# ashishkumar822/Jetson-SLAM

Hardware: AMD Instinct MI355X
Metric: stereo pairs/s (FAST+ORB extract L+R + stereo match) (higher is better)
Workload: dtype u8/int32 (+f32 orientation/blur)

## Files before the change

jetson_slam_amd/csrc/k_stereo.hip:

```cpp
#include <algorithm>
#include <cstdlib>

#include "jsorb_launch.h"

namespace jsorb {

__device__ __forceinline__ int hamming256(const uint4 a0, const uint4 a1, const uint4 b0, const uint4 b1)
{
    return __popc(a0.x ^ b0.x) + __popc(a0.y ^ b0.y) + __popc(a0.z ^ b0.z) + __popc(a0.w ^ b0.w) +
           __popc(a1.x ^ b1.x) + __popc(a1.y ^ b1.y) + __popc(a1.z ^ b1.z) + __popc(a1.w ^ b1.w);
}

#define SKPW 4
#define SGL (64 / SKPW)

__device__ __forceinline__ void wave_lds_sync_st()
{
    __builtin_amdgcn_fence(__ATOMIC_RELEASE, "wavefront");
    __builtin_amdgcn_wave_barrier();
    __builtin_amdgcn_fence(__ATOMIC_ACQUIRE, "wavefront");
}

#define ST_MAX_PASS 8
#define ST_MAX_KP (SKPW * ST_MAX_PASS)
#ifndef ST_MIN_WAVES
#define ST_MIN_WAVES 5
#endif
__global__ __launch_bounds__(64, ST_MIN_WAVES) void k_stereo(Geometry g, ImageSrc srcL, const uint8_t *slabL, ImageSrc srcR, const uint8_t *slabR,
                                               const int32_t *__restrict__ outL, const int *__restrict__ countsL, const uint8_t *__restrict__ descL,
                                               const int32_t *__restrict__ outR, const int *__restrict__ countsR, const uint8_t *__restrict__ descR,
                                               const int *__restrict__ row_tabR,
                                               float *__restrict__ u_right, float *__restrict__ depth, int *__restrict__ best_l1,
                                               unsigned *__restrict__ aux, StereoArgs sa, int n_pairs, int *__restrict__ diag, int npass)
{
    __shared__ int s_lvi[JSORB_MAX_LEVELS][12];
    __shared__ float s_lvf[JSORB_MAX_LEVELS][2];
    __shared__ unsigned s_best[ST_MAX_KP];
    __shared__ int s_ncand[ST_MAX_KP];
    __shared__ __align__(16) unsigned s_par[ST_MAX_KP][8];
    __shared__ __align__(16) unsigned s_ctr[ST_MAX_KP][4];
    __shared__ __align__(16) unsigned s_acc[ST_MAX_KP][8];
    const int lane = threadIdx.x;
    const int grp = lane / SGL, sl = lane % SGL;
    const int kpw = SKPW * npass;
    int b, blk;
    if (!xcd_map((g.T + kpw - 1) / kpw, n_pairs, b, blk)) return;
    const int Nl = uniform_i32(countsL[b * (JSORB_MAX_LEVELS + 1) + JSORB_MAX_LEVELS]);
    const int Nr = uniform_i32(countsR[b * (JSORB_MAX_LEVELS + 1) + JSORB_MAX_LEVELS]);
    if (blk * kpw >= Nl) return;
    if (lane < g.L) {
        const LevelDesc &lv = g.lv[lane];
        s_lvi[lane][3] = lv.W; s_lvi[lane][4] = lv.pitch; s_lvi[lane][5] = (int)lv.img_off;
        if (!g.epi_rows) {
            s_lvi[lane][0] = lv.th; s_lvi[lane][1] = lv.nth; s_lvi[lane][2] = lv.row_tab_off;
            s_lvi[lane][6] = (int)(0xFFFFFFFFu / (unsigned)lv.th + 1u);
            s_lvi[lane][7] = lv.tw; s_lvi[lane][8] = lv.ntw; s_lvi[lane][9] = lv.tile_off;
            s_lvi[lane][10] = (int)(0xFFFFFFFFu / (unsigned)lv.tw + 1u);
        }
        s_lvf[lane][0] = lv.scale; s_lvf[lane][1] = lv.inv_scale;
    }
    if (lane < ST_MAX_KP) { s_best[lane] = 0xFFFFFFFFu; s_ncand[lane] = 0; }
    reinterpret_cast<uint4 *>(s_acc)[lane] = make_uint4(0, 0, 0, 0);
    static_assert(ST_MAX_KP * 8 * 4 == 64 * 16, "one 16-byte store per lane clears the L1 counters");
    wave_lds_sync_st();
    const int32_t *oL = outL + (size_t)b * 6 * g.T;
    const int32_t *oR = outR + (size_t)b * 6 * g.T;
    const size_t tb = (size_t)b * g.T;

    struct LeftKp { int x, y, level; uint4 a0, a1; };
    auto load_left = [&](int pass) {
        const int i = min(blk * kpw + pass * SKPW + grp, Nl - 1);
        const uint4 *dl = reinterpret_cast<const uint4 *>(descL + (tb + i) * 32);
        return LeftKp{oL[i], oL[Nl + i], oL[4 * (size_t)Nl + i], dl[0], dl[1]};
    };
#ifndef ST_PREFETCH
#define ST_PREFETCH 1
#endif
#if ST_PREFETCH
    LeftKp nxt = load_left(0);
#endif
    for (int pass = 0; pass < npass; pass++) {
        if (blk * kpw + pass * SKPW >= Nl) break;
        const int i_raw = blk * kpw + pass * SKPW + grp;
        const bool live = i_raw < Nl;
#if ST_PREFETCH
        const LeftKp cur = nxt;
        nxt = load_left(pass + 1);
#else
        const LeftKp cur = load_left(pass);
#endif
        const int levelL = cur.level;
        const float uL = (float)cur.x, vL = (float)cur.y;
        const float minU = uL - sa.maxD, maxU = uL - 0.0f;
        unsigned best_key = 0xFFFFFFFFu;
        int n_cand = 0;
        {
            const uint4 a0 = cur.a0, a1 = cur.a1;
            const int vLi = (int)vL;
            const int *rt = row_tabR + (size_t)b * g.row_tab_stride;
            if (g.epi_rows) {
                const int EH = g.epi_rows, EN = g.L * EH;
                const int *et = rt + g.epi_off;
                const int2 *ee = reinterpret_cast<const int2 *>(et + ((EN + 2) & ~1));
                int seg_start = 0, seg_len = 0;
                {
                    const int lr = levelL - 1 + sl;
                    if (sl < 3 && lr >= 0 && lr < g.L && !(maxU < 0)) {
                        const float r = 2.0f * s_lvf[lr][0], vLf = (float)vLi;
                        const float lo_f = __builtin_floorf(vLf - 2.0f - r), hi_f = __builtin_ceilf(vLf + 2.0f + r);
                        int below = 0, above = 0;
#pragma unroll
                        for (int k = 0; k < 5; k++) {
                            below += __builtin_ceilf((lo_f + (float)k) + r) < vLf ? 1 : 0;
                            above += __builtin_floorf((hi_f - (float)k) - r) > vLf ? 1 : 0;
                        }
                        const int ylo = max((int)lo_f + below, 0), yhi = min((int)hi_f - above, EH - 1);
                        if (ylo <= yhi) {
                            seg_start = et[lr * EH + ylo];
                            seg_len = et[lr * EH + yhi + 1] - seg_start;
                        }
                    }
                }
                const int gl0 = lane & ~(SGL - 1);
                const int st0 = __shfl(seg_start, gl0, 64), st1 = __shfl(seg_start, gl0 + 1, 64), st2 = __shfl(seg_start, gl0 + 2, 64);
                const int c1 = __shfl(seg_len, gl0, 64), c2 = c1 + __shfl(seg_len, gl0 + 1, 64), total = c2 + __shfl(seg_len, gl0 + 2, 64);
#ifndef ST_CAND_UNROLL
#define ST_CAND_UNROLL 3
#endif
                constexpr int CU = ST_CAND_UNROLL;
                for (int k = sl; k < total; k += CU * SGL) {
                    int2 e[CU];
                    bool ok[CU];
#pragma unroll
                    for (int u = 0; u < CU; u++) {
                        const int kk = k + u * SGL;
                        const int kc = kk < total ? kk : k;
                        e[u] = ee[(kc >= c2 ? st2 - c2 : (kc >= c1 ? st1 - c1 : st0)) + kc];
                    }
                    uint4 b0[CU], b1[CU];
#pragma unroll
                    for (int u = 0; u < CU; u++) {
                        const float uR = (float)(e[u].y & 0xFFFF);
                        ok[u] = k + u * SGL < total && uR >= minU && uR <= maxU;
                        const uint4 *dr = reinterpret_cast<const uint4 *>(descR + (tb + (ok[u] ? e[u].x : 0)) * 32);
                        b0[u] = dr[0]; b1[u] = dr[1];
                    }
#pragma unroll
                    for (int u = 0; u < CU; u++) {
                        if (!ok[u]) continue;
                        n_cand++;
                        const int d = hamming256(a0, a1, b0[u], b1[u]);
                        if (d < sa.th_high) {
                            const unsigned key = ((unsigned)d << 20) | (unsigned)e[u].x;
                            best_key = key < best_key ? key : best_key;
                        }
                    }
                }
            } else {
            int j0[3], len[3];
            int nrw[3], tl0[3], tst[3], ncl[3];
            float rr[3];
#pragma unroll
            for (int t = 0; t < 3; t++) {
                const int lr = levelL - 1 + t;
                j0[t] = 0; len[t] = 0; rr[t] = 0.f;
                nrw[t] = 0; tl0[t] = 0; tst[t] = 0; ncl[t] = 0;
                if (lr >= 0 && lr < g.L && !(maxU < 0)) {
                    const float scl = s_lvf[lr][0], iscl = s_lvf[lr][1];
                    const int th = s_lvi[lr][0], nth = s_lvi[lr][1], rto = s_lvi[lr][2];
                    const unsigned th_magic = (unsigned)s_lvi[lr][6];
                    const float r = 2.0f * scl;
                    rr[t] = r;
                    const int lo = (int)__builtin_floorf((vL - r - 1.0f) * iscl) - 1;
                    const int hi = (int)__builtin_ceilf((vL + r + 2.0f) * iscl) + 1;
                    const int t_lo = lo < 0 ? 0 : (th > 1 ? (int)__umulhi((unsigned)lo, th_magic) : lo);
                    int t_hi = hi < 0 ? -1 : (th > 1 ? (int)__umulhi((unsigned)hi, th_magic) : hi);
                    if (t_hi > nth - 1) t_hi = nth - 1;
                    if (t_lo <= t_hi) {
                        if (!g.stereo_colprune) {
                            j0[t] = rt[rto + t_lo];
                            len[t] = rt[rto + t_hi + 1] - j0[t];
                        } else {
                            const int tw = s_lvi[lr][7], ntw = s_lvi[lr][8];
                            const unsigned tw_magic = (unsigned)s_lvi[lr][10];
                            const int xlo = (int)__builtin_floorf((minU - 1.0f) * iscl) - 1, xhi = (int)__builtin_ceilf((maxU + 1.0f) * iscl) + 1;
                            const int c_lo = xlo < 0 ? 0 : (tw > 1 ? (int)__umulhi((unsigned)xlo, tw_magic) : xlo);
                            int c_hi = xhi < 0 ? -1 : (tw > 1 ? (int)__umulhi((unsigned)xhi, tw_magic) : xhi);
                            if (c_hi > ntw - 1) c_hi = ntw - 1;
                            if (c_lo <= c_hi) {
                                nrw[t] = t_hi - t_lo + 1;
                                tl0[t] = s_lvi[lr][9] + t_lo * ntw + c_lo;
                                tst[t] = ntw;
                                ncl[t] = c_hi - c_lo + 1;
                            }
                        }
                    }
                }
            }
            auto candidate_at = [&](int j, float kpY, float uR, float r) {
                const uint4 *dr = reinterpret_cast<const uint4 *>(descR + (tb + j) * 32);
                const uint4 b0 = dr[0], b1 = dr[1];
                const int maxr = (int)__builtin_ceilf(kpY + r), minr = (int)__builtin_floorf(kpY - r);
                if (vLi < minr || vLi > maxr) return;
                if (!(uR >= minU && uR <= maxU)) return;
                n_cand++;
                const int d = hamming256(a0, a1, b0, b1);
                if (d < sa.th_high) {
                    const unsigned key = ((unsigned)d << 20) | (unsigned)j;
                    best_key = key < best_key ? key : best_key;
                }
            };
            auto candidate = [&](int j, float r) { candidate_at(j, (float)oR[Nr + j], (float)oR[j], r); };
            if (!g.stereo_colprune) {
                const int c1 = len[0], c2 = len[0] + len[1], total = c2 + len[2];
                for (int k = sl; k < total; k += SGL) {
                    const int t = k >= c2 ? 2 : (k >= c1 ? 1 : 0);
                    const int j = (t == 2 ? j0[2] - c2 : (t == 1 ? j0[1] - c1 : j0[0])) + k;
                    candidate(j, t == 2 ? rr[2] : (t == 1 ? rr[1] : rr[0]));
                }
            } else {
                const int *tp = rt + g.row_tab_len;
                const int c1 = nrw[0], c2 = nrw[0] + nrw[1], nseg = c2 + nrw[2];
                int nseg_max = nseg;
                nseg_max = max(max(__builtin_amdgcn_readlane(nseg, 0), __builtin_amdgcn_readlane(nseg, 16)),
                               max(__builtin_amdgcn_readlane(nseg, 32), __builtin_amdgcn_readlane(nseg, 48)));
                for (int s0 = 0; s0 < nseg_max; s0 += SGL) {
                    const int sg = s0 + sl;
                    int seg_start = 0, seg_len = 0;
                    float seg_r = 0.f;
                    if (sg < nseg) {
                        const int t = sg >= c2 ? 2 : (sg >= c1 ? 1 : 0);
                        const int row = sg - (t == 2 ? c2 : (t == 1 ? c1 : 0));
                        const int tile = (t == 2 ? tl0[2] : (t == 1 ? tl0[1] : tl0[0])) + row * (t == 2 ? tst[2] : (t == 1 ? tst[1] : tst[0]));
                        seg_start = tp[tile];
                        seg_len = tp[tile + (t == 2 ? ncl[2] : (t == 1 ? ncl[1] : ncl[0]))] - seg_start;
                        seg_r = t == 2 ? rr[2] : (t == 1 ? rr[1] : rr[0]);
                    }
                    const int n_here = min(SGL, nseg_max - s0);
                    for (int q = 0; q < n_here; q++) {
                        const int src_lane = (lane & ~(SGL - 1)) + q;
                        const int st = __shfl(seg_start, src_lane, 64), ln = __shfl(seg_len, src_lane, 64);
                        const float r = __shfl(seg_r, src_lane, 64);
                        for (int k = sl; k < ln; k += SGL) candidate(st + k, r);
                    }
                }
            }
            }
        }
        static_assert(SGL == 16, "the lane group of a keypoint is one DPP row");
        best_key = row16_min_u32(best_key);
        n_cand = row16_sum_i32(n_cand);
        if (live && sl == 0) { s_best[pass * SKPW + grp] = best_key; s_ncand[pass * SKPW + grp] = n_cand; }
    }
    wave_lds_sync_st();

    const int slot = lane & (ST_MAX_KP - 1);
    const int i_raw = blk * kpw + slot;
    const bool live = lane < ST_MAX_KP && slot < kpw && i_raw < Nl;
    const int i = min(i_raw, Nl - 1);
    const unsigned best_key = s_best[slot];
    const int n_cand = s_ncand[slot];
    const int xL0 = oL[i], yL0 = oL[Nl + i], levelL = oL[4 * (size_t)Nl + i];
    const float uL = (float)xL0, vL = (float)yL0;
    float out_u = -1.0f, out_d = -1.0f;
    int out_l1 = -1, corr = 0;
    const bool matched = best_key != 0xFFFFFFFFu && (int)(best_key >> 20) < sa.th_orb;
    const int bestIdxR = matched ? (int)(best_key & 0xFFFFFu) : 0;
    const float scL = s_lvf[levelL][0], iscL = s_lvf[levelL][1];
    const int WL = s_lvi[levelL][3];
    const float uR0 = (float)oR[bestIdxR];
    const float scaleduR0 = roundf(uR0 * iscL);
    const float scaleduL0 = roundf(uL * iscL);
    const float scaledvL0 = roundf(vL * iscL);
    const float iniu = scaleduR0 - 5.0f - 5.0f, endu = scaleduR0 + 5.0f + 5.0f;
    const bool refine = live && matched && !(iniu < 0 || endu >= (float)WL);
    const unsigned long long ref_mask = __ballot(refine);
    const int n_ref = __popcll(ref_mask);
    const int rank = __popcll(ref_mask & ((1ull << lane) - 1ull));
    typedef unsigned u32x4 __attribute__((ext_vector_type(4), aligned(4)));
    if (refine) {
        corr = 1;
        int pl, pr;
        const uint8_t *imL, *imR;
        if (levelL == 0) {
            pl = srcL.l0_pitch; imL = srcL.l0 + (size_t)b * srcL.l0_stride;
            pr = srcR.l0_pitch; imR = srcR.l0 + (size_t)b * srcR.l0_stride;
        } else {
            pl = pr = s_lvi[levelL][4];
            imL = slabL + (size_t)b * g.slab_bytes + (unsigned)s_lvi[levelL][5];
            imR = slabR + (size_t)b * g.slab_bytes + (unsigned)s_lvi[levelL][5];
        }
        const int xl = (int)scaleduL0, xr = (int)scaleduR0, y = (int)scaledvL0;
        const int la = (xl - 5) & ~3, ra = (xr - 10) & ~3;
        const unsigned shl = (unsigned)(xl - 5 - la), shr = (unsigned)(xr - 10 - ra);
        const uint8_t *aL = imL + (size_t)(y - 5) * pl + la, *aR = imR + (size_t)(y - 5) * pr + ra;
        const u32x4 Lq = *reinterpret_cast<const u32x4 *>(aL + (size_t)5 * pl);
        const u32x4 Rq0 = *reinterpret_cast<const u32x4 *>(aR + (size_t)5 * pr);
        const u32x4 Rq1 = *reinterpret_cast<const u32x4 *>(aR + (size_t)5 * pr + 16);
        const unsigned long long uaL = (unsigned long long)(uintptr_t)aL, uaR = (unsigned long long)(uintptr_t)aR;
        reinterpret_cast<uint4 *>(s_par[rank])[0] = make_uint4((unsigned)uaL, (unsigned)(uaL >> 32), (unsigned)uaR, (unsigned)(uaR >> 32));
        reinterpret_cast<uint4 *>(s_par[rank])[1] = make_uint4((unsigned)pl, (unsigned)pr, shl, shr);
        reinterpret_cast<uint4 *>(s_ctr[rank])[0] = make_uint4(__builtin_amdgcn_alignbyte(Lq.z, Lq.y, shl), __builtin_amdgcn_alignbyte(Rq0.z, Rq0.y, shr),
                                                               __builtin_amdgcn_alignbyte(Rq0.w, Rq0.z, shr), __builtin_amdgcn_alignbyte(Rq1.x, Rq0.w, shr));
    }
    wave_lds_sync_st();

    const int n_tasks = 11 * n_ref;
    for (int t0 = 0; t0 < n_tasks; t0 += 64) {
        const int t = t0 + lane;
        const bool mine = t < n_tasks;
        const int tt = mine ? t : 0;
        const int ridx = (tt * 745) >> 13;
        const int row = tt - 11 * ridx;
        const uint4 p0 = reinterpret_cast<const uint4 *>(s_par[ridx])[0], p1 = reinterpret_cast<const uint4 *>(s_par[ridx])[1];
        const uint4 ctr = reinterpret_cast<const uint4 *>(s_ctr[ridx])[0];
        const uint8_t *rowL = reinterpret_cast<const uint8_t *>((uintptr_t)(((unsigned long long)p0.y << 32) | p0.x)) + (size_t)row * (int)p1.x;
        const uint8_t *rowR = reinterpret_cast<const uint8_t *>((uintptr_t)(((unsigned long long)p0.w << 32) | p0.z)) + (size_t)row * (int)p1.y;
        const unsigned shl = p1.z, shr = p1.w;
        u32x4 Lq = (u32x4){0, 0, 0, 0}, Rq0 = Lq, Rq1 = Lq;
        if (mine) {
            Lq = *reinterpret_cast<const u32x4 *>(rowL);
            Rq0 = *reinterpret_cast<const u32x4 *>(rowR);
            Rq1 = *reinterpret_cast<const u32x4 *>(rowR + 16);
        }
        unsigned W[3], X[6];
        W[0] = __builtin_amdgcn_alignbyte(Lq.y, Lq.x, shl); W[1] = __builtin_amdgcn_alignbyte(Lq.z, Lq.y, shl);
        W[2] = __builtin_amdgcn_alignbyte(Lq.w, Lq.z, shl);
        X[0] = __builtin_amdgcn_alignbyte(Rq0.y, Rq0.x, shr); X[1] = __builtin_amdgcn_alignbyte(Rq0.z, Rq0.y, shr);
        X[2] = __builtin_amdgcn_alignbyte(Rq0.w, Rq0.z, shr); X[3] = __builtin_amdgcn_alignbyte(Rq1.x, Rq0.w, shr);
        X[4] = __builtin_amdgcn_alignbyte(Rq1.y, Rq1.x, shr); X[5] = __builtin_amdgcn_alignbyte(Rq1.z, Rq1.y, shr);
        const unsigned cW1 = ctr.x, cX1 = ctr.y, cX2 = ctr.z, cX3 = ctr.w;
        const unsigned cX[4] = {0u, cX1, cX2, cX3};
        const int lc = (int)((cW1 >> 8) & 0xFFu);
        unsigned A[6], E[11], O[10];
#pragma unroll
        for (int m = 0; m < 6; m++)
            A[m] = __builtin_amdgcn_perm(0u, W[m >> 1], (m & 1) ? 0x0c030c02u : 0x0c010c00u) + 0x01000100u;
        A[5] &= 0x0000FFFFu;
#pragma unroll
        for (int m = 0; m < 11; m++) E[m] = __builtin_amdgcn_perm(0u, X[m >> 1], (m & 1) ? 0x0c030c02u : 0x0c010c00u);
#pragma unroll
        for (int m = 0; m < 10; m++)
            O[m] = (m & 1) ? __builtin_amdgcn_perm(X[(m + 1) >> 1], X[(m - 1) >> 1], 0x0c040c03u) : __builtin_amdgcn_perm(0u, X[m >> 1], 0x0c020c01u);
        unsigned part[12];
        part[11] = 0;
#pragma unroll
        for (int q = 0; q < 11; q++) {
            const int rc = (int)((cX[(5 + q) >> 2] >> (8 * ((5 + q) & 3))) & 0xFFu);
            const unsigned kv = (unsigned)(lc - rc + 256);
            const unsigned kpk = (kv << 16) | kv;
            unsigned pq_ = 0;
#pragma unroll
            for (int m = 0; m < 6; m++) {
                typedef unsigned short us2 __attribute__((ext_vector_type(2)));
                const unsigned Rp = (q & 1) ? O[(q >> 1) + m] : E[(q >> 1) + m];
                unsigned Bp = __builtin_bit_cast(unsigned, (us2)(__builtin_bit_cast(us2, Rp) + __builtin_bit_cast(us2, kpk)));
                if (m == 5) Bp &= 0x0000FFFFu;
                pq_ = __builtin_amdgcn_sad_u16(A[m], Bp, pq_);
            }
            part[q] = pq_;
        }
        if (mine) {
#pragma unroll
            for (int q2 = 0; q2 < 6; q2++) atomicAdd(&s_acc[ridx][q2], part[2 * q2] | (part[2 * q2 + 1] << 16));
        }
    }
    wave_lds_sync_st();

    int acc[11];
    {
        const uint4 a0 = reinterpret_cast<const uint4 *>(s_acc[refine ? rank : 0])[0], a1 = reinterpret_cast<const uint4 *>(s_acc[refine ? rank : 0])[1];
        acc[0] = (int)(a0.x & 0xFFFFu); acc[1] = (int)(a0.x >> 16); acc[2] = (int)(a0.y & 0xFFFFu); acc[3] = (int)(a0.y >> 16);
        acc[4] = (int)(a0.z & 0xFFFFu); acc[5] = (int)(a0.z >> 16); acc[6] = (int)(a0.w & 0xFFFFu); acc[7] = (int)(a0.w >> 16);
        acc[8] = (int)(a1.x & 0xFFFFu); acc[9] = (int)(a1.x >> 16); acc[10] = (int)(a1.y & 0xFFFFu);
    }
    if (refine) {
        unsigned kmin = ((unsigned)acc[0] << 4);
#pragma unroll
        for (int s = 1; s < 11; s++) kmin = min(kmin, ((unsigned)acc[s] << 4) | (unsigned)s);
        const int bestDist = (int)(kmin >> 4), bestR = (int)(kmin & 15u);
        if (!(bestR == 0 || bestR == 10)) {
            float dist1 = 0.f, dist2 = 0.f, dist3 = 0.f;
#pragma unroll
            for (int s = 1; s < 10; s++)
                if (s == bestR) { dist1 = (float)acc[s - 1]; dist2 = (float)acc[s]; dist3 = (float)acc[s + 1]; }
            const float deltaR = (dist1 - dist3) / (2.0f * (dist1 + dist3 - 2.0f * dist2));
            if (!(deltaR < -1 || deltaR > 1)) {
                float bestuR = scL * ((scaleduR0 + (float)bestR - 5.0f) + deltaR);
                float disparity = uL - bestuR;
                if (disparity >= 0.0f && disparity < sa.maxD) {
                    if (disparity <= 0) {
                        disparity = 0.01f;
                        bestuR = (float)((double)uL - 0.01);
                    }
                    out_d = sa.mbf / disparity;
                    out_u = bestuR;
                    out_l1 = bestDist;
                }
            }
        }
    }
    if (live) {
        u_right[tb + i] = out_u;
        depth[tb + i] = out_d;
        best_l1[tb + i] = out_l1;
        aux[tb + i] = (n_cand & 0x7FFFFFFF) | (corr ? 0x80000000u : 0u);
        if (diag) {
            int *dg = diag + (size_t)(tb + i) * JSORB_STEREO_DIAG_INTS;
            const int bd = best_key == 0xFFFFFFFFu ? 0x7FFFFFFF : (int)(best_key >> 20);
            dg[0] = bd < sa.th_high ? (int)(best_key & 0xFFFFFu) : -1;
            dg[1] = bd < sa.th_high ? bd : sa.th_high;
#pragma unroll
            for (int q = 0; q < 11; q++) dg[2 + q] = corr ? acc[q] : -1;
        }
    }
}


__device__ __forceinline__ int block256_exclusive_scan(int v, int *s_w, int &total)
{
    const int tid = threadIdx.x, lane = tid & 63, wave = uniform_i32(tid >> 6);
    const int incl = wave_inclusive_scan_i32(v);
    if (lane == 63) s_w[wave] = incl;
    __syncthreads();
    const int w0 = s_w[0], w1 = s_w[1], w2 = s_w[2], w3 = s_w[3];
    total = w0 + w1 + w2 + w3;
    const int base = wave == 0 ? 0 : wave == 1 ? w0 : wave == 2 ? w0 + w1 : w0 + w1 + w2;
    __syncthreads();
    return base + incl - v;
}

#define MED_BIN_SHIFT 8
static_assert((2 * 5 + 1) * (2 * 5 + 1) * 510 < (256 << MED_BIN_SHIFT), "L1 distance range exceeds the first-level histogram");

struct MedianShared {
    int hist[4][256];
    int sel[4];
    int s_w[4];
    int s_cand, s_corr, s_removed;
};

template <class ForEach>
__device__ __forceinline__ float median_threshold(MedianShared &sm, int tid, ForEach for_each, int &nv_out)
{
    const int wave = uniform_i32(tid >> 6);
    for_each([&](int d) { if (d >= 0) atomicAdd(&sm.hist[wave][d >> MED_BIN_SHIFT], 1); });
    __syncthreads();
    int nv;
    {
        const int h = sm.hist[0][tid] + sm.hist[1][tid] + sm.hist[2][tid] + sm.hist[3][tid];
        const int excl = block256_exclusive_scan(h, sm.s_w, nv);
        const int kth = nv / 2;
        if (h > 0 && excl <= kth && kth < excl + h) { sm.sel[0] = tid; sm.sel[1] = kth - excl; }
    }
    nv_out = nv;
    if (nv == 0) return 3.0e38f;
    __syncthreads();
#pragma unroll
    for (int w = 0; w < 4; w++) sm.hist[w][tid] = 0;
    __syncthreads();
    const int bin = sm.sel[0], kin = sm.sel[1];
    for_each([&](int d) { if (d >= 0 && (d >> MED_BIN_SHIFT) == bin) atomicAdd(&sm.hist[wave][d & ((1 << MED_BIN_SHIFT) - 1)], 1); });
    __syncthreads();
    {
        const int h = sm.hist[0][tid] + sm.hist[1][tid] + sm.hist[2][tid] + sm.hist[3][tid];
        int tot;
        const int excl = block256_exclusive_scan(h, sm.s_w, tot);
        if (h > 0 && excl <= kin && kin < excl + h) sm.sel[3] = (bin << MED_BIN_SHIFT) | tid;
    }
    __syncthreads();
    const float median = (float)sm.sel[3];
    return 1.5f * 1.4f * median;
}

__device__ __noinline__ void median_big(MedianShared &sm, const Geometry &g, const int *__restrict__ countsL, float *__restrict__ u_right,
                                        float *__restrict__ depth, const int *__restrict__ best_l1,
                                        const unsigned *__restrict__ aux, int *__restrict__ stats, DeliverStereo dl)
{
    const int tid = threadIdx.x, b = blockIdx.x;
    const int Nl = countsL[b * (JSORB_MAX_LEVELS + 1) + JSORB_MAX_LEVELS];
    const size_t tb = (size_t)b * g.T;
    int *st = stats + b * 8;
    int cand = 0, corr = 0;
    for (int i = tid; i < Nl; i += 256) {
        const unsigned a = aux[tb + i];
        cand += (int)(a & 0x7FFFFFFFu);
        corr += (int)(a >> 31);
    }
    cand = wave_sum_i32(cand);
    corr = wave_sum_i32(corr);
    if ((tid & 63) == 0) { atomicAdd(&sm.s_cand, cand); atomicAdd(&sm.s_corr, corr); }
    int nv;
    const float thDist = median_threshold(sm, tid, [&](auto f) { for (int i = tid; i < Nl; i += 256) f(best_l1[tb + i]); }, nv);
    int removed = 0;
    for (int i = tid; i < Nl; i += 256) {
        const int d = best_l1[tb + i];
        float u = -1.0f, z = -1.0f;
        if (dl.u_host) { u = u_right[tb + i]; z = depth[tb + i]; }
        if (d >= 0 && !((float)d < thDist)) {
            u = -1.0f; z = -1.0f;
            u_right[tb + i] = u;
            depth[tb + i] = z;
            removed++;
        }
        if (dl.u_host) { dl.u_host[i] = u; dl.d_host[i] = z; }
    }
    if (removed) atomicAdd(&sm.s_removed, removed);
    __syncthreads();
    if (tid == 0) {
        const int v[4] = {sm.s_cand, sm.s_corr, nv, nv - sm.s_removed};
#pragma unroll
        for (int k = 0; k < 4; k++) { st[k] = v[k]; if (dl.stats_host) dl.stats_host[b * 8 + k] = v[k]; }
    }
}

template <int MED_R>
__global__ __launch_bounds__(256) void k_median(Geometry g, const int *__restrict__ countsL, float *__restrict__ u_right,
                                                float *__restrict__ depth, const int *__restrict__ best_l1,
                                                const unsigned *__restrict__ aux, int *__restrict__ stats, DeliverStereo dl)
{
    __shared__ MedianShared sm;
    const int tid = threadIdx.x, b = blockIdx.x;
    const int Nl = countsL[b * (JSORB_MAX_LEVELS + 1) + JSORB_MAX_LEVELS];
    const size_t tb = (size_t)b * g.T;
    int *st = stats + b * 8;
#pragma unroll
    for (int w = 0; w < 4; w++) sm.hist[w][tid] = 0;
    if (tid == 0) { sm.s_cand = 0; sm.s_corr = 0; sm.s_removed = 0; }
    __syncthreads();
    if (Nl > 256 * MED_R) {
        median_big(sm, g, countsL, u_right, depth, best_l1, aux, stats, dl);
        return;
    }
    int d[MED_R];
    int cand = 0, corr = 0;
#pragma unroll
    for (int r = 0; r < MED_R; r++) {
        const int i = tid + 256 * r;
        d[r] = -1;
        if (i < Nl) {
            d[r] = best_l1[tb + i];
            const unsigned a = aux[tb + i];
            cand += (int)(a & 0x7FFFFFFFu);
            corr += (int)(a >> 31);
        }
    }
    float uu[MED_R], zz[MED_R];
    if (dl.u_host) {
#pragma unroll
        for (int r = 0; r < MED_R; r++) {
            const int i = tid + 256 * r;
            uu[r] = -1.0f; zz[r] = -1.0f;
            if (i < Nl) { uu[r] = u_right[tb + i]; zz[r] = depth[tb + i]; }
        }
    }
    cand = wave_sum_i32(cand);
    corr = wave_sum_i32(corr);
    if ((tid & 63) == 0) { atomicAdd(&sm.s_cand, cand); atomicAdd(&sm.s_corr, corr); }
    int nv;
    const float thDist = median_threshold(sm, tid, [&](auto f) {
#pragma unroll
        for (int r = 0; r < MED_R; r++) f(d[r]);
    }, nv);
    int removed = 0;
#pragma unroll
    for (int r = 0; r < MED_R; r++) {
        const int i = tid + 256 * r;
        const bool cut = d[r] >= 0 && !((float)d[r] < thDist);
        if (cut) {
            u_right[tb + i] = -1.0f;
            depth[tb + i] = -1.0f;
            removed++;
        }
        if (dl.u_host && i < Nl) { dl.u_host[i] = cut ? -1.0f : uu[r]; dl.d_host[i] = cut ? -1.0f : zz[r]; }
    }
    if (removed) atomicAdd(&sm.s_removed, removed);
    __syncthreads();
    if (tid == 0) {
        const int v[4] = {sm.s_cand, sm.s_corr, nv, nv - sm.s_removed};
#pragma unroll
        for (int k = 0; k < 4; k++) { st[k] = v[k]; if (dl.stats_host) dl.stats_host[b * 8 + k] = v[k]; }
    }
}

__global__ void k_gather_counts(const int *__restrict__ countsL, const int *__restrict__ countsR, const int *__restrict__ stats,
                                int32_t *__restrict__ dst, int n_pairs)
{
    const int b = blockIdx.x * blockDim.x + threadIdx.x;
    if (b >= n_pairs) return;
    dst[3 * b + 0] = countsL[b * (JSORB_MAX_LEVELS + 1) + JSORB_MAX_LEVELS];
    dst[3 * b + 1] = countsR[b * (JSORB_MAX_LEVELS + 1) + JSORB_MAX_LEVELS];
    dst[3 * b + 2] = stats[b * 8 + 3];
}

void launch_gather_counts(const int *countsL, const int *countsR, const int *stats, int32_t *dst, int n_pairs, hipStream_t s)
{
    hipLaunchKernelGGL(k_gather_counts, dim3((n_pairs + 255) / 256), dim3(256), 0, s, countsL, countsR, stats, dst, n_pairs);
}

void launch_stereo(const Geometry &g, const ImageSrc &srcL, const uint8_t *slabL, const ImageSrc &srcR, const uint8_t *slabR,
                   const int32_t *outL, const int *countsL, const uint8_t *descL,
                   const int32_t *outR, const int *countsR, const uint8_t *descR, const int *row_tabR,
                   float *u_right, float *depth, int *best_l1, unsigned *aux, StereoArgs a, int n_pairs, hipStream_t s, int *diag)
{
    static const int env_pass = experiment_env("JSORB_STEREO_PASSES") ? std::max(1, std::min(ST_MAX_PASS, atoi(experiment_env("JSORB_STEREO_PASSES")))) : 0;
    auto waves = [&](int np) { return (long)n_pairs * ((g.T + SKPW * np - 1) / (SKPW * np)); };
    int npass = 1;
    if (env_pass) npass = env_pass;
    else if (n_pairs > 1) npass = waves(8) >= 24576 ? 8 : waves(6) >= 12288 ? 6 : waves(4) >= 12288 ? 4 : waves(2) >= 12288 ? 2 : 1;
    const int kpw = SKPW * npass;
    hipLaunchKernelGGL(k_stereo, xcd_grid((g.T + kpw - 1) / kpw, n_pairs), dim3(64), 0, s, g, srcL, slabL, srcR, slabR, outL, countsL, descL,
                       outR, countsR, descR, row_tabR, u_right, depth, best_l1, aux, a, n_pairs, diag, npass);
}

void launch_median(const Geometry &g, const int *countsL, float *u_right, float *depth, const int *best_l1, const unsigned *aux,
                   int *stats, int n_pairs, hipStream_t s, DeliverStereo dl)
{
    if (g.T <= 256 * 32) hipLaunchKernelGGL(k_median<32>, dim3(n_pairs), dim3(256), 0, s, g, countsL, u_right, depth, best_l1, aux, stats, dl);
    else hipLaunchKernelGGL(k_median<64>, dim3(n_pairs), dim3(256), 0, s, g, countsL, u_right, depth, best_l1, aux, stats, dl);
}

}
```

Baseline: 135,900.

## Precompute epipolar segments per block and software-pipeline stereo candidate loads

Loads every left keypoint's coordinates once at kernel start into LDS and computes all epipolar row segments in two wave-wide passes, replacing the per-pass segment computation and shuffles. Candidate entries for the next pass are prefetched while the current pass issues its descriptor requests. The winning right-keypoint x is recorded in LDS during scoring, so the refine stage no longer gathers it from global memory. This costs more LDS and registers, which may lower occupancy, and the argmin tie handling for the stored uR has to stay consistent with the packed key.

```diff
diff --git a/jetson_slam_amd/csrc/k_stereo.hip b/jetson_slam_amd/csrc/k_stereo.hip
--- a/jetson_slam_amd/csrc/k_stereo.hip
+++ b/jetson_slam_amd/csrc/k_stereo.hip
@@ -37,6 +37,9 @@
     __shared__ float s_lvf[JSORB_MAX_LEVELS][2];
     __shared__ unsigned s_best[ST_MAX_KP];
     __shared__ int s_ncand[ST_MAX_KP];
+    __shared__ int s_uR[ST_MAX_KP];
+    __shared__ int s_kp[3][ST_MAX_KP];
+    __shared__ __align__(8) int s_seg[ST_MAX_KP][6];
     __shared__ __align__(16) unsigned s_par[ST_MAX_KP][8];
     __shared__ __align__(16) unsigned s_ctr[ST_MAX_KP][4];
     __shared__ __align__(16) unsigned s_acc[ST_MAX_KP][8];
@@ -48,6 +51,20 @@
     const int Nl = uniform_i32(countsL[b * (JSORB_MAX_LEVELS + 1) + JSORB_MAX_LEVELS]);
     const int Nr = uniform_i32(countsR[b * (JSORB_MAX_LEVELS + 1) + JSORB_MAX_LEVELS]);
     if (blk * kpw >= Nl) return;
+    const int32_t *oL = outL + (size_t)b * 6 * g.T;
+    const int32_t *oR = outR + (size_t)b * 6 * g.T;
+    const size_t tb = (size_t)b * g.T;
+    const int slot = lane & (ST_MAX_KP - 1);
+    const int i_raw = blk * kpw + slot;
+    const int i = min(i_raw, Nl - 1);
+    const int kx0 = oL[i], ky0 = oL[Nl + i], klv0 = oL[4 * (size_t)Nl + i];
+    struct LeftDesc { uint4 a0, a1; };
+    auto load_left = [&](int pass) {
+        const int il = min(blk * kpw + pass * SKPW + grp, Nl - 1);
+        const uint4 *dl = reinterpret_cast<const uint4 *>(descL + (tb + il) * 32);
+        return LeftDesc{dl[0], dl[1]};
+    };
+    LeftDesc nxt = load_left(0);
     if (lane < g.L) {
         const LevelDesc &lv = g.lv[lane];
         s_lvi[lane][3] = lv.W; s_lvi[lane][4] = lv.pitch; s_lvi[lane][5] = (int)lv.img_off;
@@ -59,92 +76,101 @@
         }
         s_lvf[lane][0] = lv.scale; s_lvf[lane][1] = lv.inv_scale;
     }
-    if (lane < ST_MAX_KP) { s_best[lane] = 0xFFFFFFFFu; s_ncand[lane] = 0; }
+    if (lane < ST_MAX_KP) {
+        s_best[lane] = 0xFFFFFFFFu; s_ncand[lane] = 0; s_uR[lane] = 0;
+        s_kp[0][lane] = kx0; s_kp[1][lane] = ky0; s_kp[2][lane] = klv0;
+    }
     reinterpret_cast<uint4 *>(s_acc)[lane] = make_uint4(0, 0, 0, 0);
     static_assert(ST_MAX_KP * 8 * 4 == 64 * 16, "one 16-byte store per lane clears the L1 counters");
     wave_lds_sync_st();
-    const int32_t *oL = outL + (size_t)b * 6 * g.T;
-    const int32_t *oR = outR + (size_t)b * 6 * g.T;
-    const size_t tb = (size_t)b * g.T;
-
-    struct LeftKp { int x, y, level; uint4 a0, a1; };
-    auto load_left = [&](int pass) {
-        const int i = min(blk * kpw + pass * SKPW + grp, Nl - 1);
-        const uint4 *dl = reinterpret_cast<const uint4 *>(descL + (tb + i) * 32);
-        return LeftKp{oL[i], oL[Nl + i], oL[4 * (size_t)Nl + i], dl[0], dl[1]};
-    };
-#ifndef ST_PREFETCH
-#define ST_PREFETCH 1
-#endif
-#if ST_PREFETCH
-    LeftKp nxt = load_left(0);
-#endif
-    for (int pass = 0; pass < npass; pass++) {
-        if (blk * kpw + pass * SKPW >= Nl) break;
-        const int i_raw = blk * kpw + pass * SKPW + grp;
-        const bool live = i_raw < Nl;
-#if ST_PREFETCH
-        const LeftKp cur = nxt;
-        nxt = load_left(pass + 1);
-#else
-        const LeftKp cur = load_left(pass);
-#endif
-        const int levelL = cur.level;
-        const float uL = (float)cur.x, vL = (float)cur.y;
-        const float minU = uL - sa.maxD, maxU = uL - 0.0f;
-        unsigned best_key = 0xFFFFFFFFu;
-        int n_cand = 0;
-        {
-            const uint4 a0 = cur.a0, a1 = cur.a1;
-            const int vLi = (int)vL;
-            const int *rt = row_tabR + (size_t)b * g.row_tab_stride;
-            if (g.epi_rows) {
-                const int EH = g.epi_rows, EN = g.L * EH;
-                const int *et = rt + g.epi_off;
-                const int2 *ee = reinterpret_cast<const int2 *>(et + ((EN + 2) & ~1));
-                int seg_start = 0, seg_len = 0;
-                {
-                    const int lr = levelL - 1 + sl;
-                    if (sl < 3 && lr >= 0 && lr < g.L && !(maxU < 0)) {
-                        const float r = 2.0f * s_lvf[lr][0], vLf = (float)vLi;
-                        const float lo_f = __builtin_floorf(vLf - 2.0f - r), hi_f = __builtin_ceilf(vLf + 2.0f + r);
-                        int below = 0, above = 0;
-#pragma unroll
-                        for (int k = 0; k < 5; k++) {
-                            below += __builtin_ceilf((lo_f + (float)k) + r) < vLf ? 1 : 0;
-                            above += __builtin_floorf((hi_f - (float)k) - r) > vLf ? 1 : 0;
-                        }
-                        const int ylo = max((int)lo_f + below, 0), yhi = min((int)hi_f - above, EH - 1);
-                        if (ylo <= yhi) {
-                            seg_start = et[lr * EH + ylo];
-                            seg_len = et[lr * EH + yhi + 1] - seg_start;
-                        }
-                    }
+    const int *rt = row_tabR + (size_t)b * g.row_tab_stride;
+    const int *et = rt + g.epi_off;
+    const int2 *ee = reinterpret_cast<const int2 *>(et + ((g.L * g.epi_rows + 2) & ~1));
+    if (g.epi_rows) {
+        const int EH = g.epi_rows;
+        const float maxU = (float)kx0 - 0.0f, vL = (float)ky0;
+        const int vLi = (int)vL;
+        int lo_i[2], hi_i[2];
+        bool task[2], has[2];
+#pragma unroll
+        for (int it = 0; it < 2; it++) {
+            const int lr = klv0 - 1 + (it == 0 ? (lane >> 5) : 2);
+            task[it] = slot < kpw && (it == 0 || lane < ST_MAX_KP);
+            has[it] = false; lo_i[it] = 0; hi_i[it] = 0;
+            if (task[it] && lr >= 0 && lr < g.L && !(maxU < 0)) {
+                const float r = 2.0f * s_lvf[lr][0], vLf = (float)vLi;
+                const float lo_f = __builtin_floorf(vLf - 2.0f - r), hi_f = __builtin_ceilf(vLf + 2.0f + r);
+                int below = 0, above = 0;
+#pragma unroll
+                for (int k = 0; k < 5; k++) {
+                    below += __builtin_ceilf((lo_f + (float)k) + r) < vLf ? 1 : 0;
+                    above += __builtin_floorf((hi_f - (float)k) - r) > vLf ? 1 : 0;
                 }
-                const int gl0 = lane & ~(SGL - 1);
-                const int st0 = __shfl(seg_start, gl0, 64), st1 = __shfl(seg_start, gl0 + 1, 64), st2 = __shfl(seg_start, gl0 + 2, 64);
-                const int c1 = __shfl(seg_len, gl0, 64), c2 = c1 + __shfl(seg_len, gl0 + 1, 64), total = c2 + __shfl(seg_len, gl0 + 2, 64);
+                const int ylo = max((int)lo_f + below, 0), yhi = min((int)hi_f - above, EH - 1);
+                if (ylo <= yhi) { has[it] = true; lo_i[it] = lr * EH + ylo; hi_i[it] = lr * EH + yhi + 1; }
+            }
+        }
+        int seg_start[2], seg_end[2];
+#pragma unroll
+        for (int it = 0; it < 2; it++) {
+            seg_start[it] = has[it] ? et[lo_i[it]] : 0;
+            seg_end[it] = has[it] ? et[hi_i[it]] : 0;
+        }
+#pragma unroll
+        for (int it = 0; it < 2; it++)
+            if (task[it]) *reinterpret_cast<int2 *>(&s_seg[slot][2 * (it == 0 ? (lane >> 5) : 2)]) = make_int2(seg_start[it], seg_end[it] - seg_start[it]);
+        wave_lds_sync_st();
+    }
+
 #ifndef ST_CAND_UNROLL
 #define ST_CAND_UNROLL 3
 #endif
-                constexpr int CU = ST_CAND_UNROLL;
-                for (int k = sl; k < total; k += CU * SGL) {
-                    int2 e[CU];
-                    bool ok[CU];
-#pragma unroll
-                    for (int u = 0; u < CU; u++) {
-                        const int kk = k + u * SGL;
-                        const int kc = kk < total ? kk : k;
-                        e[u] = ee[(kc >= c2 ? st2 - c2 : (kc >= c1 ? st1 - c1 : st0)) + kc];
-                    }
-                    uint4 b0[CU], b1[CU];
+    constexpr int CU = ST_CAND_UNROLL;
+    struct Runs { int st0, st1, st2, c1, c2, total; };
+    auto runs_of = [&](int pass) {
+        const int2 *sg = reinterpret_cast<const int2 *>(s_seg[pass * SKPW + grp]);
+        const int2 r0 = sg[0], r1 = sg[1], r2 = sg[2];
+        return Runs{r0.x, r1.x, r2.x, r0.y, r0.y + r1.y, r0.y + r1.y + r2.y};
+    };
+    auto load_entries = [&](const Runs &rn, int k, int2 (&e)[CU]) {
+#pragma unroll
+        for (int u = 0; u < CU; u++) {
+            const int kk = k + u * SGL;
+            e[u] = make_int2(0, 0);
+            if (kk < rn.total) e[u] = ee[(kk >= rn.c2 ? rn.st2 - rn.c2 : (kk >= rn.c1 ? rn.st1 - rn.c1 : rn.st0)) + kk];
+        }
+    };
+    int2 nxt_e[CU];
+#pragma unroll
+    for (int u = 0; u < CU; u++) nxt_e[u] = make_int2(0, 0);
+    if (g.epi_rows) load_entries(runs_of(0), sl, nxt_e);
+    for (int pass = 0; pass < npass; pass++) {
+        if (blk * kpw + pass * SKPW >= Nl) break;
+        const bool live = blk * kpw + pass * SKPW + grp < Nl;
+        const bool more = pass + 1 < npass && blk * kpw + (pass + 1) * SKPW < Nl;
+        const LeftDesc cur = nxt;
+        if (more) nxt = load_left(pass + 1);
+        const float uL = (float)s_kp[0][pass * SKPW + grp];
+        const float minU = uL - sa.maxD, maxU = uL - 0.0f;
+        unsigned best_key = 0xFFFFFFFFu;
+        int n_cand = 0, best_uR = 0;
+        {
+            const uint4 a0 = cur.a0, a1 = cur.a1;
+            if (g.epi_rows) {
+                const Runs rn = runs_of(pass);
+                int2 e[CU];
+                bool ok[CU];
+                uint4 b0[CU], b1[CU];
+                auto request = [&](int k) {
 #pragma unroll
                     for (int u = 0; u < CU; u++) {
                         const float uR = (float)(e[u].y & 0xFFFF);
-                        ok[u] = k + u * SGL < total && uR >= minU && uR <= maxU;
+                        ok[u] = k + u * SGL < rn.total && uR >= minU && uR <= maxU;
                         const uint4 *dr = reinterpret_cast<const uint4 *>(descR + (tb + (ok[u] ? e[u].x : 0)) * 32);
                         b0[u] = dr[0]; b1[u] = dr[1];
                     }
+                };
+                auto score = [&]() {
 #pragma unroll
                     for (int u = 0; u < CU; u++) {
                         if (!ok[u]) continue;
@@ -152,11 +178,24 @@
                         const int d = hamming256(a0, a1, b0[u], b1[u]);
                         if (d < sa.th_high) {
                             const unsigned key = ((unsigned)d << 20) | (unsigned)e[u].x;
-                            best_key = key < best_key ? key : best_key;
+                            if (key < best_key) { best_key = key; best_uR = e[u].y & 0xFFFF; }
                         }
                     }
+                };
+#pragma unroll
+                for (int u = 0; u < CU; u++) e[u] = nxt_e[u];
+                request(sl);
+                if (more) load_entries(runs_of(pass + 1), sl, nxt_e);
+                score();
+                for (int k = sl + CU * SGL; k < rn.total; k += CU * SGL) {
+                    load_entries(rn, k, e);
+                    request(k);
+                    score();
                 }
             } else {
+            const int levelL = s_kp[2][pass * SKPW + grp];
+            const float vL = (float)s_kp[1][pass * SKPW + grp];
+            const int vLi = (int)vL;
             int j0[3], len[3];
             int nrw[3], tl0[3], tst[3], ncl[3];
             float rr[3];
@@ -248,19 +287,17 @@
             }
         }
         static_assert(SGL == 16, "the lane group of a keypoint is one DPP row");
-        best_key = row16_min_u32(best_key);
+        const unsigned grp_key = row16_min_u32(best_key);
         n_cand = row16_sum_i32(n_cand);
-        if (live && sl == 0) { s_best[pass * SKPW + grp] = best_key; s_ncand[pass * SKPW + grp] = n_cand; }
+        if (live && sl == 0) { s_best[pass * SKPW + grp] = grp_key; s_ncand[pass * SKPW + grp] = n_cand; }
+        if (live && best_key == grp_key && grp_key != 0xFFFFFFFFu) s_uR[pass * SKPW + grp] = best_uR;
     }
     wave_lds_sync_st();
 
-    const int slot = lane & (ST_MAX_KP - 1);
-    const int i_raw = blk * kpw + slot;
     const bool live = lane < ST_MAX_KP && slot < kpw && i_raw < Nl;
-    const int i = min(i_raw, Nl - 1);
     const unsigned best_key = s_best[slot];
     const int n_cand = s_ncand[slot];
-    const int xL0 = oL[i], yL0 = oL[Nl + i], levelL = oL[4 * (size_t)Nl + i];
+    const int xL0 = s_kp[0][slot], yL0 = s_kp[1][slot], levelL = s_kp[2][slot];
     const float uL = (float)xL0, vL = (float)yL0;
     float out_u = -1.0f, out_d = -1.0f;
     int out_l1 = -1, corr = 0;
@@ -268,7 +305,7 @@
     const int bestIdxR = matched ? (int)(best_key & 0xFFFFFu) : 0;
     const float scL = s_lvf[levelL][0], iscL = s_lvf[levelL][1];
     const int WL = s_lvi[levelL][3];
-    const float uR0 = (float)oR[bestIdxR];
+    const float uR0 = (float)(g.epi_rows ? s_uR[slot] : oR[bestIdxR]);
     const float scaleduR0 = roundf(uR0 * iscL);
     const float scaleduL0 = roundf(uL * iscL);
     const float scaledvL0 = roundf(vL * iscL);
@@ -603,7 +640,8 @@
                    const int32_t *outR, const int *countsR, const uint8_t *descR, const int *row_tabR,
                    float *u_right, float *depth, int *best_l1, unsigned *aux, StereoArgs a, int n_pairs, hipStream_t s, int *diag)
 {
-    static const int env_pass = experiment_env("JSORB_STEREO_PASSES") ? std::max(1, std::min(ST_MAX_PASS, atoi(experiment_env("JSORB_STEREO_PASSES")))) : 0;
+    const char *env_str = experiment_env("JSORB_STEREO_PASSES");
+    const int env_pass = env_str ? std::max(1, std::min(ST_MAX_PASS, atoi(env_str))) : 0;
     auto waves = [&](int np) { return (long)n_pairs * ((g.T + SKPW * np - 1) / (SKPW * np)); };
     int npass = 1;
     if (env_pass) npass = env_pass;
```

After: 136,700 (median of 6 runs). No clear change (+0.6%).
